# rhasspy/piper

Hardware: AMD Instinct MI355X
Metric: audio samples/sec (higher is better)
Workload: dtype f32

## Files before the change

### piper_amd/csrc/engine.h

```cpp
#pragma once
#include <cstdint>
#include <deque>
#include <list>
#include <map>
#include <string>
#include <unordered_map>
#include <vector>

#include "pe_rt.h"
#include "kernels/params.h"
#include "policy.h"
#include "weights.h"

namespace pe {

struct PackedConv {
  float* wp = nullptr;
  float* wp16 = nullptr;
  float* wpb = nullptr;
  const float* wunscale = nullptr;
  float* wpg4 = nullptr;
  float* bias = nullptr;
  int rows = 0;
  int mtiles = 0;
// ... 178 lines not shown
  int H_, C_, FC_, nh_, dk_, nlayers_, ksz_, window_, hop_, U_;
  std::vector<void*> owned_;
  size_t weight_bytes_ = 0;

  float* emb_ = nullptr;
  float* emb_g_ = nullptr;
  struct EncLayer {
    PackedConv qkv, o, f1, f2;
    float* o16 = nullptr;
    float* qkv16 = nullptr;
    const float *f1p = nullptr, *f2p = nullptr;
    float *relk, *relv, *g1, *b1, *g2, *b2;
  };
  std::vector<EncLayer> enc_;
  PackedConv enc_proj_;
  float* enc_proj16_ = nullptr;
  PackedConv dp_pre_, dp_proj_;
  DdsW dp_dds_;
  struct CFlow {
    float *pre_w, *pre_b;
    DdsW dds;
    PackedConv proj;
    float* proj16 = nullptr;
  };
  std::vector<CFlow> cflows_;
  float ea_m0_ = 0, ea_es0_ = 1;
  float *ea_dev_m_ = nullptr, *ea_dev_logs_ = nullptr;
 public:
  void arena_ready();
 private:
  struct Rcl {
    PackedConv pre, post;
    float *pre16 = nullptr, *post16 = nullptr;
    const float* pre4pad = nullptr;
    std::vector<PackedConv> in, rs;
    std::vector<const float*> rs4;
    int in_off, out_off;
  };
  std::vector<Rcl> rcls_;
  PackedConv dec_pre_;
  struct UpStage {
    PackedConv up;
    int rate, ch;
    std::vector<std::vector<PackedConv>> rb;
    float* last_bias_sum = nullptr;
    struct HostConv { std::vector<float> w; int co = 0, ci = 0, k = 0, dil = 1; const float* bias = nullptr; };
    std::vector<std::vector<HostConv>> rb_host;
    void* mrf_phases = nullptr; float* mrf_w = nullptr;
    float* mrf_wsplit = nullptr; float* mrf_unscale = nullptr; int mrf_wsplit_floats = 0;
    int mrf_wfloats = 0, mrf_cp = 0, mrf_hx = 0;
    std::vector<struct MrfPhase> mrf_ph;
    bool mrf_ok = false, mrf_rb1 = false;
  };
  struct MrfGeo { int ou = 0, N = 0, cu_lo = 0, cu_hi = 0, nleft = 0, nhalo = 0; };
  bool mrf_geo(const UpStage& st, int len_mul, bool tail, MrfGeo& best) const;
  void build_mrf(UpStage& st);
  void mrf(const UpStage& st, View x, View out, const int* lens, int len_mul, int Lmax, bool tail = false);
  bool matrix_bf3_ = false, pack_bf3_now_ = false;
  int matrix_sm_ = 0;
  static bool env_bf3();
 public:
  bool matrix_bf3() const { return matrix_bf3_; }
  int matrix_split_mode() const { return matrix_bf3_ ? matrix_sm_ : -1; }
 private:
  std::vector<UpStage> ups_;
  float* post_w_ = nullptr;
  int post_cin_ = 0;
  struct CondW { float* w; float* b; int rows; };
  CondW cond_dp_{nullptr, nullptr, 0}, cond_dec_{nullptr, nullptr, 0};
  std::vector<CondW> cond_wn_;
  int gin_ = 0, nspk_ = 1;

  int B_ = 0, Tmax_ = 0, Ts_ = 0, Fmax_ = 0, Fs_ = 0, Tg_ = 0, Fg_ = 0;
  bool use_graphs_ = true;
  struct GraphEntry { std::string key; void* exec; long launches; };
  std::list<GraphEntry> graphs_;
  std::unordered_map<std::string, std::list<GraphEntry>::iterator> graph_of_;
  long graph_captures_ = 0;
 public:
  long graph_captures() const { return graph_captures_; }
  size_t graphs_cached() const { return graphs_.size(); }
  static int id_bucket(int T);
  static int frame_bucket(int F);
  void warmup(int max_batch, int max_ids, float frames_per_id, const float* scales, const int64_t* sample, int64_t n_sample);
 private:
  long run_launches_ = 0;
  unsigned long long* d_rng_ = nullptr;
  float scales_[3] = {0.667f, 1.0f, 0.8f};
  std::vector<float> spec_rel_;
  float spec_rel(int b) const { return (size_t)b < spec_rel_.size() ? spec_rel_[b] : 1.f; }
  bool have_noise_w_ = false, have_noise_z_ = false;
  bool drew_w_ = false;
  bool fold_dur_ = false;
  DurP fold_dp_{};
  std::vector<int64_t> id_off_;
  std::vector<int32_t> tlens_h_, frames_h_, dur_h_;
  std::vector<int64_t> sample_off_;
  uint64_t seed_ = 1234, call_ = 0;
  const float* h_noise_z_ = nullptr;
  int64_t h_noise_z_stride_ = 0;

  size_t capA_B_ = 0, capA_T_ = 0, capB_B_ = 0, capB_F_ = 0;
  bool capB_exact_ = false;
  size_t ws_budget_ = 0;
  size_t ws_budget();
  char* wsA_ = nullptr; size_t wsA_bytes_ = 0;
  char* wsB_ = nullptr; size_t wsB_bytes_ = 0;
  int *d_ids_ = nullptr, *d_tlens_ = nullptr, *d_sids_ = nullptr, *d_dur_ = nullptr, *d_cum_ = nullptr,
// ... 56 lines not shown
```

### piper_amd/csrc/engine_launch.cpp

```cpp
#include "engine_internal.h"

namespace pe {


bool Engine::can_group(const PackedConv& pc, int ncols) const {
  if (stage_tiled_) return false;
  const long blocks = (long)((ncols + CFG_BN[pc.cfg] - 1) / CFG_BN[pc.cfg]) * (pc.mtiles * 32 / CFG_BM[pc.cfg]) * B_;
  return pol_.groupable(pc.gate, pc.up != 0, blocks, (pc.ntaps - 1) * pc.dil, pc.Cin);
}
bool Engine::can_group_tiled(const PackedConv& pc, int ncols) const {
  return !pc.gate && pc.up == 0 && route(pc, ncols, EPI_STORE) == ROUTE_TILE && !(matrix_bf3_ && pc.wpb) &&
         !pol_.one_tap_direct(pc.gate, false, pc.ntaps, pc.Cin) && (pc.ntaps - 1) * pc.dil <= 128;
}
static int tile_cfg_of(int cfg) { return cfg == CFG_C ? CFG_C : CFG_S; }
void Engine::group_begin(bool tiled) {
  grouping_ = true;
  group_tiled_ = tiled;
  group_cfg_ = -1;
  group_.clear();
  group_flops_ = group_bytes_ = 0;
}
void Engine::group_end() {
  grouping_ = false;
  if (group_.empty()) return;
// ... 206 lines not shown
    const int BM = BF3_BM[bc], BN = BF3_BN[bc];
    const int HALO = p.xhalo <= 64 ? 64 : 128;
    const int nbuf = pc.nchunks == 1 ? 1 : 2;
    const int nterm = matrix_sm_ == 2 ? 3 : 2;
    const size_t smem = (size_t)nbuf * nterm * 64 * ((BN + HALO + 63) / 64 * 64);
    dim3 grid((ncols + BN - 1) / BN, pc.mtiles * 32 / BM, B_);
    int kh = -1;
    if (prof_level_ >= 2) {
      char nm[96];
      snprintf(nm, sizeof(nm), "conv_split_kernel<%d,%s,%s,%d>", matrix_sm_, (pc.gate && bc == 1) ? "1,4,2,1" : bnames[bc],
               pc.gate ? "true" : "false", HALO);
      kh = kbegin(krow(std::string(nm)), kflops, kbytes);
    }
    launch::conv_bf3(matrix_sm_, bc, pc.gate, HALO, grid, smem, ls_, p);
    kend(kh);
    return;
  }
  if (pol_.one_tap_direct(pc.gate, epi == EPI_CONVT, pc.ntaps, pc.Cin)) {
    const dim3 grid((ncols + 63) / 64, (pc.mtiles + 1) / 2, B_);
    int kh = -1;
    if (prof_level_ >= 2) {
      char nm[96];
      int n = snprintf(nm, sizeof(nm), "conv1x1_kernel<1>");
      if (pol_.prof_sites) snprintf(nm + n, sizeof(nm) - n, "|%dx%dx%d e%d L%d", pc.rows, pc.Cin, pc.ntaps, epi, len_mul);
      kh = kbegin(krow(std::string(nm)), kflops, kbytes);
    }
    launch::conv1x1(grid, ls_, p);
    kend(kh);
    return;
  }
  if (cfg == CFG_A) cfg = pc.gate ? CFG_G : CFG_S;
  else if (cfg == CFG_B && !pc.gate) cfg = CFG_S;
  const int BM = CFG_BM[cfg], BN = CFG_BN[cfg];
  const int ntile = (ncols + BN - 1) / BN, mblocks = pc.mtiles * 32 / BM;
  const int tpb = pol_.tiles_per_workgroup();
  p.tpb = tpb;
  dim3 grid((ntile + tpb - 1) / tpb, mblocks, B_);
  if (p.xhalo > 128) throw std::runtime_error("conv halo (kernel-1)*dilation > 128 is not supported");
  const int nbuf = (tpb == 1 && pc.nchunks == 1) ? 1 : 2;
  const int HALO = p.xhalo <= 64 ? 64 : 128;
  const size_t smem = (size_t)nbuf * KC * ((BN + HALO + 63) / 64 * 64) * sizeof(float);
  static const char* knames[] = {"2,2,2,2,8", "1,4,2,1,16", "1,4,1,1,16", "2,2,1,1,16", "2,2,2,1,16", "1,4,1,2,16", "1,4,2,2,8"};
  int kh = -1;
  if (prof_level_ >= 2) {
    char nm[96];
    int n = snprintf(nm, sizeof(nm), "conv_mfma_kernel<%s,%s,%d>", knames[cfg], pc.gate ? "true" : "false", HALO);
    if (pol_.prof_sites) snprintf(nm + n, sizeof(nm) - n, "|%dx%dx%d d%d e%d L%d", pc.rows, pc.Cin, pc.ntaps, pc.dil, epi, len_mul);
    kh = kbegin(krow(std::string(nm)), kflops, kbytes);
  }
  launch::conv_tile(cfg, pc.gate, HALO, grid, smem, ls_, p);
  kend(kh);
}

bool Engine::mrf_geo(const UpStage& st, int len_mul, bool tail, MrfGeo& best) const {
  const int CP = st.mrf_cp, NCG = CP == 32 ? 8 : 4, HU = CP == 32 ? 1 : 2;
  const int OUMAX = CP == 32 ? 4 : 3;
  const int hx = st.mrf_hx, hxa = rup(hx, 16);
  auto geo = [&](int ou, MrfGeo& g) {
    g.ou = ou; g.N = 16 * NCG * ou;
    if (hxa + g.N + hx > mrf_ws(CP, ou)) return false;
    g.cu_lo = (hxa - hx) / 16; g.cu_hi = (hxa + g.N + hx + 15) / 16;
    g.nleft = hxa / 16 - g.cu_lo; g.nhalo = g.cu_hi - g.cu_lo - g.N / 16;
    return g.nhalo <= NCG * HU;
  };
  best = MrfGeo{};
  double best_cost = 0;
  MrfGeo forced;
  const int force = (pol_.mrf_ou >= 1 && pol_.mrf_ou <= OUMAX && geo((int)pol_.mrf_ou, forced)) ? (int)pol_.mrf_ou : 0;
  for (int ou = 1; ou <= OUMAX; ++ou) {
    MrfGeo g;
    if ((force && ou != force) || !geo(ou, g)) continue;
    double wgs = 0;
    const int stride = tail ? g.N - (POST_K - 1) : g.N;
    for (int b = 0; b < B_; ++b) wgs += (double)(((long)frames_h_[b] * len_mul + stride - 1) / stride);
    double work = 0, taps = 0;
    for (auto& P : st.mrf_ph) {
      const int lo = (hxa - P.e) / 16, hi = (hxa + g.N + P.e + 15) / 16;
      work += (double)(hi - lo) * 16 * P.ntaps;
      taps += P.ntaps;
    }
    double cost = std::ceil(wgs / 256.0) * (work + 16.0 * taps);
    if (ou == 4) cost *= 1.06;
    if (!best.ou || cost < best_cost) { best = g; best_cost = cost; }
  }
  return best.ou != 0;
}

void Engine::mrf(const UpStage& st, View x, View out, const int* lens, int len_mul, int Lmax, bool tail) {
  const int CP = st.mrf_cp, HU = CP == 32 ? 1 : 2;
  const int hx = st.mrf_hx, hxa = rup(hx, 16);
  MrfGeo best;
  if (!mrf_geo(st, len_mul, tail, best)) throw std::runtime_error("internal: no mrf_kernel geometry for this stage");
  MrfP p{};
  p.x = x.p; p.x_bs = x.bs; p.x_cs = x.cs;
  p.out = out.p; p.o_bs = out.bs; p.o_cs = out.cs;
  p.lens = lens; p.len_mul = len_mul;
  p.phases = static_cast<const MrfPhase*>(st.mrf_phases); p.nphases = (int)st.mrf_ph.size();
  p.wstream = st.mrf_w; p.wfloats = st.mrf_wfloats;
  p.C = st.ch; p.N = best.N; p.wcols = hxa + best.N + hx; p.hxa = hxa; p.cu_lo = best.cu_lo; p.cu_hi = best.cu_hi;
  p.nleft = best.nleft; p.nhalo = best.nhalo;
  p.slope = 0.1f;
  p.alpha = 1.0f / (float)st.rb.size();
  p.stride = best.N; p.n0off = 0;
  p.post_w = nullptr; p.audio = nullptr; p.a_bs = 0; p.absmax = nullptr; p.post_slope = 0.01f;
  if (tail) {
    p.stride = best.N - (POST_K - 1); p.n0off = (POST_K - 1) / 2;
    p.post_w = post_w_; p.audio = audio_; p.a_bs = Ss_; p.absmax = absmax_;
  }
  double kflops = 0, kbytes = 0;
  if (prof_level_ >= 2) {
    double cols = 0;
    for (int b = 0; b < B_; ++b) cols += (double)frames_h_[b] * len_mul;
    double macs = 0;
    for (auto& cv : st.rb)
      for (auto& c : cv) macs += c.macs_per_col;
    kflops = 2.0 * macs * cols;
    kbytes = 8.0 * st.ch * cols + 4.0 * st.mrf_wfloats;
    if (tail) {
      kflops += 2.0 * cols * st.ch * POST_K;
      kbytes = 4.0 * (st.ch + 1) * cols + 4.0 * st.mrf_wfloats;
    }
  }
  dim3 grid((Lmax + p.stride - 1) / p.stride, B_);
  char nm[64];
  const bool split = matrix_bf3_ && pol_.mrf_split && st.mrf_wsplit != nullptr && matrix_sm_ < 2;
  if (split) {
    p.wstream = st.mrf_wsplit; p.wfloats = st.mrf_wsplit_floats; p.wunscale = st.mrf_unscale;
    snprintf(nm, sizeof(nm), "mrf_split_kernel<%d,%d,%d,%d>", matrix_sm_, CP, best.ou, HU);
  } else {
    snprintf(nm, sizeof(nm), "mrf_kernel<%d,%d,%d>", CP, best.ou, HU);
  }
  const int kh = prof_level_ >= 2 ? kbegin(krow(std::string(nm)), kflops, kbytes) : -1;
  if (split) launch::mrf_split(matrix_sm_, CP, best.ou, grid, ls_, p);
  else launch::mrf(CP, best.ou, grid, ls_, p);
  kend(kh);
}

size_t Engine::attn_smem(int T, bool global_scores) const {
  const int SP = rup(T, 64) + 1, VS = dk_ + 1 + (dk_ & 1);
  return ((global_scores ? 0 : (size_t)ATT_QB * SP) + (size_t)ATT_KCH * VS + (size_t)dk_ * ATT_QB +
          (size_t)2 * (2 * window_ + 1) * dk_ + 4 * ATT_QB * 16) * sizeof(float);
}
bool Engine::attn_scores_global(int T) const { return pol_.attn_long || attn_smem(T, false) > (size_t)160 * 1024; }

void Engine::layer_norm(View in, View out, const float* g, const float* b, int C, const int* lens, int Lmax) {
  LnP p;
  p.in = in.p; p.i_bs = in.bs; p.i_cs = in.cs;
  p.out = out.p; p.o_bs = out.bs; p.o_cs = out.cs;
  p.gamma = g; p.beta = b;
  p.lens = lens; p.C = C;
  if (C > LN_COLS * 32) throw std::runtime_error("LayerNorm over more than 256 channels is not supported");
  dim3 grid((Lmax + LN_COLS - 1) / LN_COLS, B_);
  const int kh = kbegin(prof_level_ >= 2 ? krow("ln_kernel") : 0, 0.0, 4.0 * 2.0 * C * (lens == d_tlens_ ? cols_ids_ : cols_frames_));
  launch::layer_norm(grid, stream_, p);
  kend(kh);
}

void Engine::dds_params(const DdsW& d, View in, View out, View tmp, const DdsOpt* opt, std::vector<DdsP>& list) {
  int dil = 1;
  const int n = (int)d.c1x1.size();
  View cur = in;
  for (int i = 0; i < n; ++i) {
    const View dst = ((n - 1 - i) & 1) ? tmp : out;
    if (dst.p == cur.p) throw std::runtime_error("internal: DDSConv buffer aliasing");
    DdsP p{};
    if (opt && i == 0 && opt->pre_z) {
      p.pre_z = opt->pre_z; p.pre_z_bs = opt->pre_z_bs; p.pre_w = opt->pre_w; p.pre_b = opt->pre_b;
    }
    p.z_scale = opt ? opt->z_scale : nullptr;
    if (opt && i == n - 1 && opt->post_w16) {
      p.post_w16 = opt->post_w16; p.post_w4 = w4_of(opt->post_w16); p.post_bias = opt->post_bias; p.post_rows = opt->post_rows;
      p.post_out = opt->post_out.p; p.po_bs = opt->post_out.bs; p.po_cs = opt->post_out.cs;
      p.zin = opt->zin; p.zin_bs = opt->zin_bs; p.z_cs = opt->z_cs; p.c0 = opt->c0; p.c1 = opt->c1;
      p.zout = opt->zout; p.zout_bs = opt->zout_bs;
      p.inv_sqrt_h = 1.0f / std::sqrt((float)H_);
    }
    p.x = cur.p; p.x_bs = cur.bs; p.x_cs = cur.cs;
    p.out = dst.p; p.o_bs = dst.bs; p.o_cs = dst.cs;
// ... 193 lines not shown
```

### piper_amd/csrc/kernels/mrf.h

```cpp
#pragma once
#include "../pe_rt.h"
#include "params.h"
#include "conv_common.h"

namespace pe {

template <int V> struct pe_int { static constexpr int value = V; };



template <int NVM, int NDS, int K>
__device__ __forceinline__ void mrf_interleave() {
  if constexpr (NVM + NDS > 0) {
    PE_SCHED_GROUP(0x8, K);
    if constexpr (NVM > 0) {
      PE_SCHED_GROUP(0x20, 1);
      mrf_interleave<NVM - 1, NDS, K>();
    } else {
      PE_SCHED_GROUP(0x100, 1);
      mrf_interleave<0, NDS - 1, K>();
    }
  }
}

// ... 22 lines not shown
  const int l15 = lane & 15, lq = lane >> 4;
  const int ms0 = (wv % NRG) * MSW, cg = wv / NRG;
  const int g0 = n0 - p.hxa;
  const float slope = p.slope;
  const int C = p.C;
  const int wcols = p.wcols;

  const pe_rowsrc wd = pe_make_row(p.wstream, p.wfloats);
  const int wlane = ms0 * 512 + lane * 4;
  const int wlast = PE_UNIFORM(p.wfloats - STEPF);
  auto load_a = [&](int woff, f32x4 (&a)[MSW][2]) {
    woff = woff < wlast ? woff : wlast;
#pragma unroll
    for (int m = 0; m < MSW; ++m)
#pragma unroll
      for (int q = 0; q < 2; ++q) a[m][q] = pe_row_load4_so(wd, wlane + (m * 2 + q) * 256, woff);
  };
  f32x4 aA[MSW][2], aB[MSW][2];
  int wnext = 0;
  load_a(wnext, aA);
  wnext += STEPF;
  {
    const int* gp = reinterpret_cast<const int*>(p.phases);
    for (int i = tid; i < p.nphases * 12; i += NT) tph[i] = gp[i];
    if (tid < MRF_PAD) { sm[tid] = 0.f; bufs[2 * bufsz + tid] = 0.f; }
  }

  const float* xb = p.x + (long)b * p.x_bs;
  auto stage_x = [&]() {
    constexpr int NCC = (WS + 63) / 64, RPW = CP / NW;
    float v[RPW][NCC];
#pragma unroll
    for (int i = 0; i < RPW; ++i) {
      const int row = wv + NW * i;
      const pe_rowsrc rd = pe_make_row(xb + (long)row * p.x_cs, row < C ? L : 0);
#pragma unroll
      for (int j = 0; j < NCC; ++j) v[i][j] = pe_row_load(rd, (lane + 64 * j < wcols) ? g0 + lane + 64 * j : -1);
    }
#pragma unroll
    for (int i = 0; i < RPW; ++i)
#pragma unroll
      for (int j = 0; j < NCC; ++j) {
        const int c = lane + 64 * j;
        if (c < WS) bufs[(wv + NW * i) * WS + c] = pe_lrelu(v[i][j], slope);
      }
  };

  f32x4 acc[MSW][UPW], rawc[MSW][UPW], tot[MSW][OU];
  int cu[UPW];
  {
    const int cuo0 = p.hxa / 16, nout = p.N / 16;
#pragma unroll
    for (int u = 0; u < OU; ++u) cu[u] = cuo0 + cg + NCG * u;
#pragma unroll
    for (int v = 0; v < HU; ++v) {
      const int h = cg + NCG * v;
      cu[OU + v] = h >= p.nhalo ? -1 : (h < p.nleft ? p.cu_lo + h : cuo0 + nout + (h - p.nleft));
    }
#pragma unroll
    for (int m = 0; m < MSW; ++m) {
#pragma unroll
      for (int u = 0; u < UPW; ++u)
#pragma unroll
        for (int r = 0; r < 4; ++r) rawc[m][u][r] = 0.f;
#pragma unroll
      for (int u = 0; u < OU; ++u)
#pragma unroll
        for (int r = 0; r < 4; ++r) tot[m][u][r] = 0.f;
    }
  }
  const pe_rowsrc xd = pe_make_row(xb, C * p.x_cs);
  constexpr int SK = CP == 64 ? 6 : 7;
  PE_STAMP(SK, 0);
  stage_x();
  PE_STAMP(SK, 1);

  for (int ph = 0; ph < p.nphases; ++ph) {
    __syncthreads();
    MrfPhase P;
    {
      const int* t = tph + ph * 12;
      const unsigned lo = PE_UNIFORM((unsigned)t[0]), hi = PE_UNIFORM((unsigned)t[1]);
      P.bias = reinterpret_cast<const float*>(((unsigned long long)hi << 32) | lo);
      P.ntaps = PE_UNIFORM(t[2]); P.dil = PE_UNIFORM(t[3]); P.e = PE_UNIFORM(t[4]);
      P.src = PE_UNIFORM(t[5]); P.dst = PE_UNIFORM(t[6]); P.flags = PE_UNIFORM(t[7]);
    }
    if (P.flags & MRF_RESTAGE) {
      stage_x();
      __syncthreads();
    }
    if (P.flags & MRF_INIT) {
#pragma unroll
      for (int u = 0; u < UPW; ++u) {
        const int g = g0 + 16 * cu[u] + l15;
        int voff = (cu[u] >= 0 && g >= 0 && g < L) ? 4 * lq * p.x_cs + g : 0x3fffffff;
        PE_OPAQUE(voff);
#pragma unroll
        for (int m = 0; m < MSW; ++m) {
          const int vm = (C == CP || (ms0 + m) * 16 + 4 * lq < C) ? voff : 0x3fffffff;
#pragma unroll
          for (int r = 0; r < 4; ++r) rawc[m][u][r] = pe_row_load_so(xd, vm, ((ms0 + m) * 16 + r) * p.x_cs);
        }
      }
    }
    const pe_rowsrc bd = pe_make_row(P.bias, P.bias ? C : 0);
    float bz[MSW][4];
#pragma unroll
    for (int m = 0; m < MSW; ++m)
#pragma unroll
      for (int r = 0; r < 4; ++r) bz[m][r] = pe_row_load(bd, (ms0 + m) * 16 + 4 * lq + r);
    const int hh = P.dil * (P.ntaps - 1) / 2;
    const int wlo = p.hxa - P.e, whi = p.hxa + p.N + P.e;
    bool act[UPW];
#pragma unroll
    for (int u = 0; u < UPW; ++u) {
      act[u] = cu[u] >= 0 && 16 * cu[u] < whi && 16 * cu[u] + 16 > wlo;
#pragma unroll
      for (int m = 0; m < MSW; ++m)
#pragma unroll
        for (int r = 0; r < 4; ++r) acc[m][u][r] = 0.f;
    }
    const float* src = bufs + P.src * bufsz;
    if (ph < 7) PE_STAMP(SK, 2 + 3 * ph);
    auto k_loop = [&](auto maskc) {
      constexpr int MASK = decltype(maskc)::value;
      const int nsteps = NCH * P.ntaps;
      const float* ub[UPW];
#pragma unroll
      for (int u = 0; u < UPW; ++u) ub[u] = src + lq * WS + l15 + 16 * (cu[u] < 0 ? 0 : cu[u]) - hh;
      auto read_b = [&](int soff, float (&bv)[UPW][8]) {
#pragma unroll
        for (int u = 0; u < UPW; ++u)
          if (u < OU || ((MASK >> (u - OU)) & 1)) {
            const float* bp = ub[u] + soff;
#pragma unroll
            for (int s8 = 0; s8 < 8; ++s8) bv[u][s8] = bp[4 * s8 * WS];
          }
      };
      auto mma = [&](const f32x4 (&a)[MSW][2], const float (&bv)[UPW][8]) {
#pragma unroll
        for (int s8 = 0; s8 < 8; ++s8)
#pragma unroll
          for (int u = 0; u < UPW; ++u)
            if (u < OU || ((MASK >> (u - OU)) & 1)) {
#pragma unroll
              for (int m = 0; m < MSW; ++m) acc[m][u] = pe_mfma_16x16x4(a[m][s8 >> 2][s8 & 3], bv[u][s8], acc[m][u]);
            }
      };
      int ntap = 0, nchunk = 0;
      auto advance = [&]() -> int {
        if (++ntap == P.ntaps) { ntap = 0; if (++nchunk == NCH) nchunk = 0; }
        return PE_UNIFORM(nchunk * KC * WS + ntap * P.dil);
      };
      constexpr int NU = OU + ((MASK & 1) ? 1 : 0) + ((MASK & 2) ? 1 : 0);
      constexpr int NMF = 8 * MSW * NU, NVM = 2 * MSW, NDS = 4 * NU;
      if constexpr (MRF_HALF_B<CP, OU, HU>::value) {
        auto read_bh = [&](int soff, int h, float (&bv)[UPW][4]) {
#pragma unroll
          for (int u = 0; u < UPW; ++u)
            if (u < OU || ((MASK >> (u - OU)) & 1)) {
              const float* bp = ub[u] + soff;
#pragma unroll
              for (int s4 = 0; s4 < 4; ++s4) bv[u][s4] = bp[4 * (4 * h + s4) * WS];
            }
        };
        auto mma_h = [&](const f32x4 (&a)[MSW][2], int h, const float (&bv)[UPW][4]) {
#pragma unroll
          for (int s4 = 0; s4 < 4; ++s4)
#pragma unroll
            for (int u = 0; u < UPW; ++u)
              if (u < OU || ((MASK >> (u - OU)) & 1)) {
#pragma unroll
                for (int m = 0; m < MSW; ++m) acc[m][u] = pe_mfma_16x16x4(a[m][h][s4], bv[u][s4], acc[m][u]);
              }
        };
        constexpr int KH0 = (NMF / 2) / (NVM + NDS / 2 + 1), KH1 = (NMF / 2) / (NDS / 2 + 1);
        float b0[UPW][4], b1[UPW][4];
        int cur = 0;
        read_bh(0, 0, b0);
        int st = 0;
        for (; st + 1 < nsteps; st += 2) {
          PE_SCHED_FENCE();
          load_a(wnext, aB);
          read_bh(cur, 1, b1);
          wnext += STEPF;
          mma_h(aA, 0, b0);
          mrf_interleave<NVM, NDS / 2, KH0>();
          PE_SCHED_FENCE();
          cur = advance();
          read_bh(cur, 0, b0);
          mma_h(aA, 1, b1);
          mrf_interleave<0, NDS / 2, KH1>();
          PE_SCHED_FENCE();
          load_a(wnext, aA);
          read_bh(cur, 1, b1);
          wnext += STEPF;
          mma_h(aB, 0, b0);
          mrf_interleave<NVM, NDS / 2, KH0>();
          PE_SCHED_FENCE();
          cur = advance();
          read_bh(cur, 0, b0);
          mma_h(aB, 1, b1);
          mrf_interleave<0, NDS / 2, KH1>();
          PE_SCHED_FENCE();
        }
        if (st < nsteps) {
          load_a(wnext, aB);
          read_bh(cur, 1, b1);
          wnext += STEPF;
          mma_h(aA, 0, b0);
          mrf_interleave<NVM, NDS / 2, KH0>();
          PE_SCHED_FENCE();
          mma_h(aA, 1, b1);
          PE_SCHED_FENCE();
#pragma unroll
          for (int m = 0; m < MSW; ++m)
#pragma unroll
            for (int q = 0; q < 2; ++q) aA[m][q] = aB[m][q];
        }
      } else {
      constexpr int KI = NMF / (NVM + NDS + 1);
      float bA[UPW][8], bB[UPW][8];
      read_b(0, bA);
      int st = 0;
      for (; st + 1 < nsteps; st += 2) {
        PE_SCHED_FENCE();
        load_a(wnext, aB);
        read_b(advance(), bB);
        wnext += STEPF;
        mma(aA, bA);
        mrf_interleave<NVM, NDS, KI>();
        PE_SCHED_FENCE();
        load_a(wnext, aA);
        read_b(advance(), bA);
        wnext += STEPF;
        mma(aB, bB);
        mrf_interleave<NVM, NDS, KI>();
        PE_SCHED_FENCE();
      }
      if (st < nsteps) {
        load_a(wnext, aB);
        wnext += STEPF;
        mma(aA, bA);
        mrf_interleave<NVM, 0, KI>();
        PE_SCHED_FENCE();
#pragma unroll
        for (int m = 0; m < MSW; ++m)
#pragma unroll
          for (int q = 0; q < 2; ++q) aA[m][q] = aB[m][q];
      }
      }
    };
    {
      int mask = 0;
#pragma unroll
      for (int v = 0; v < HU; ++v) mask |= act[OU + v] ? (1 << v) : 0;
      mask = PE_UNIFORM(mask);
      if (HU == 1) {
        if (mask) k_loop(pe_int<1>{}); else k_loop(pe_int<0>{});
      } else {
        switch (mask) {
          case 0: k_loop(pe_int<0>{}); break;
          case 1: k_loop(pe_int<1>{}); break;
          case 2: k_loop(pe_int<2>{}); break;
          default: k_loop(pe_int<3>{}); break;
        }
      }
    }
    if (ph < 7) PE_STAMP(SK, 3 + 3 * ph);
    float* dstb = bufs + (P.dst < 0 ? 0 : P.dst) * bufsz;
#pragma unroll
    for (int u = 0; u < UPW; ++u)
      if (act[u]) {
        const int col = 16 * cu[u] + l15;
        const int g = g0 + col;
        const bool inside = g >= 0 && g < L;
#pragma unroll
        for (int m = 0; m < MSW; ++m) {
          f32x4 v;
#pragma unroll
          for (int r = 0; r < 4; ++r) {
            float t = acc[m][u][r] + bz[m][r];
            if (P.flags & MRF_RES) t += rawc[m][u][r];
            v[r] = inside ? t : 0.f;
          }
          if (P.flags & MRF_KEEP) rawc[m][u] = v;
          if (u < OU && (P.flags & MRF_FINAL)) {
#pragma unroll
            for (int r = 0; r < 4; ++r) tot[m][u < OU ? u : 0][r] += v[r];
          }
          if (P.dst >= 0) {
#pragma unroll
            for (int r = 0; r < 4; ++r) dstb[((ms0 + m) * 16 + 4 * lq + r) * WS + col] = pe_lrelu(v[r], slope);
          }
        }
        if (ph == 4 && u < 4) PE_STAMP(SK, 20 + u);
      }
    if (ph < 7) PE_STAMP(SK, 4 + 3 * ph);
  }
  if (p.post_w == nullptr) {
    float* ob = p.out + (long)b * p.o_bs;
#pragma unroll
    for (int u = 0; u < OU; ++u) {
      const int g = g0 + 16 * cu[u] + l15;
      if (g >= L) continue;
#pragma unroll
      for (int m = 0; m < MSW; ++m)
#pragma unroll
        for (int r = 0; r < 4; ++r) {
          const int row = (ms0 + m) * 16 + 4 * lq + r;
          if (row < C) ob[(long)row * p.o_cs + g] = tot[m][u][r] * p.alpha;
        }
    }
    return;
  }
  __syncthreads();
  float* mb = bufs;
  float* part = bufs + bufsz;
#pragma unroll
  for (int u = 0; u < OU; ++u) {
    const int col = 16 * cu[u] + l15;
#pragma unroll
    for (int m = 0; m < MSW; ++m)
#pragma unroll
      for (int r = 0; r < 4; ++r) mb[((ms0 + m) * 16 + 4 * lq + r) * WS + col] = pe_lrelu(tot[m][u][r] * p.alpha, p.post_slope);
  }
  __syncthreads();
  static_assert(POST_CG * POST_CU == 32 && POST_OPT == 4 && POST_K == 7, "tail mapping: 4 channel groups x 128 threads x 4 samples");
  const int nsamp = p.N - (POST_K - 1);
  {
    const int pg = PE_UNIFORM(tid >> 7), ct = tid & 127;
    if (4 * ct < nsamp) {
      float a4[POST_OPT];
#pragma unroll
      for (int o = 0; o < POST_OPT; ++o) a4[o] = 0.f;
#pragma unroll
      for (int cc = 0; cc < POST_CU; ++cc) {
        const int c = pg * POST_CU + cc;
        if (c < C) {
          const float* rp = mb + c * WS + p.hxa + 4 * ct;
          const f32x4 v0 = *reinterpret_cast<const f32x4*>(rp), v1 = *reinterpret_cast<const f32x4*>(rp + 4);
          const float v[POST_OPT + POST_K - 1] = {v0[0], v0[1], v0[2], v0[3], v1[0], v1[1], v1[2], v1[3], rp[8], rp[9]};
          const float* wc = p.post_w + c * POST_K;
#pragma unroll
          for (int k = 0; k < POST_K; ++k) {
            const float wk = wc[k];
#pragma unroll
            for (int o = 0; o < POST_OPT; ++o) a4[o] = fmaf(wk, v[o + k], a4[o]);
          }
        }
      }
#pragma unroll
      for (int o = 0; o < POST_OPT; ++o) part[pg * p.N + 4 * ct + o] = a4[o];
    }
  }
  __syncthreads();
  float pk = 0.f;
  if (tid < nsamp) {
    float sum = 0.f;
#pragma unroll
    for (int g = 0; g < POST_CG; ++g) sum += part[g * p.N + tid];
    const float y = tanhf(sum);
    const int n = n0 + (POST_K - 1) / 2 + tid;
    if (n < L) {
      p.audio[(long)b * p.a_bs + n] = y;
      pk = fabsf(y);
    }
  }
  for (int o = 32; o >= 1; o >>= 1) pk = fmaxf(pk, __shfl_xor(pk, o));
  float* wmax = part + POST_CG * p.N;
  if (lane == 0) wmax[wv] = pk;
  __syncthreads();
  if (tid == 0) {
    float m = wmax[0];
// ... 8 lines not shown
```

### piper_amd/csrc/kernels/params.h

```cpp
#pragma once
#include <cstddef>

namespace pe {

static constexpr int KC = 32;
enum Epi { EPI_STORE = 0, EPI_RESADD = 1, EPI_GATE = 2, EPI_WNRS = 3, EPI_SUBFROM = 4,
           EPI_ACCUM = 5, EPI_CONVT = 6 };
enum Act { ACT_NONE = 0, ACT_RELU = 1 };
struct ConvP {
  const float* x; long x_bs; int x_cs;
  const float* wp;
  const float* wp16;
  const float* wpb;
  const float* wunscale;
  const float* wpg4;
  const float* bias;
  const float* bias2; int bias2_bs;
  float* out; long o_bs; int o_cs;
  const float* res; long r_bs; int r_cs;
  float* out2; long o2_bs; int o2_cs;
  const int* lens; int len_mul;
  int Cin, rows;
  int nchunks;
  int ntaps, dil, padl;
// ... 131 lines not shown
  const unsigned long long* h_rng; const int* h_lens; const int* h_sids; const float* h_scales; const int* h_ids;
  int* d_lens; int* d_sids; float* d_scales;
  float* draw_out; long draw_stride; int draw_rows, draw_cols;
};

static constexpr int MAX_FRAMES = 60000;
struct DurP {
  const float* z0; long z_bs; float m0, es0;
  const float* scales;
  const int* lens; int* dur; int* cum; int d_bs; int* frames; float* logw_out;
  int* frames_host; int* frames_clamped; int frame_cap;
};
static constexpr int RNG_PITCH = 65536;
static inline unsigned randn_blocks(long rows, int cols) { return (unsigned)(rows * ((cols + 1023) / 1024)); }
struct RegP {
  const float* stats; long s_bs; int s_cs;
  const int* cum; int d_bs;
  const int* tlens; const int* frames;
  float* noise; long n_bs; int n_cs;
  const float* scales;
  float* out; long o_bs; int o_cs;
  int C;
  unsigned* absmax;
  const unsigned long long* rng; int gen;
  DurP dur; int fold;
};
static constexpr int REG_MAXT = 4096;

static constexpr int POST_K = 7, POST_OPT = 4, POST_CU = 8, POST_CG = 4, POST_SPB = 64 * POST_OPT;

enum { MRF_RES = 1, MRF_KEEP = 2, MRF_FINAL = 4, MRF_INIT = 8, MRF_RESTAGE = 16 };
struct MrfPhase {
  const float* bias;
  int ntaps, dil;
  int e;
  int src, dst;
  int flags;
  int pad[4];
};
static_assert(sizeof(MrfPhase) == 48, "MrfPhase is read as 12 ints");
struct MrfP {
  const float* x; long x_bs; int x_cs;
  float* out; long o_bs; int o_cs;
  const int* lens; int len_mul;
  const MrfPhase* phases; int nphases;
  const float* wstream; int wfloats;
  const float* wunscale;
  int C;
  int N;
  int wcols;
  int hxa;
  int cu_lo, cu_hi;
  int nleft, nhalo;
  float slope, alpha;
  int stride, n0off;
  const float* post_w; float* audio; long a_bs; unsigned* absmax; float post_slope;
};
static constexpr int MRF_NW = 8, MRF_PAD = 128, MRF_MAXPH = 24;
static constexpr int mrf_ws(int cp, int ou = 1) { return cp == 32 ? (ou >= 4 ? 624 : 528) : 304; }
static constexpr size_t mrf_smem_bytes(int cp, int ou = 1) {
  return ((size_t)2 * MRF_PAD + (size_t)2 * cp * mrf_ws(cp, ou) + MRF_MAXPH * 12) * sizeof(float);
}

}
```

### piper_amd/csrc/policy.cpp

```cpp
#include "policy.h"

#include <cerrno>
#include <cstdio>
#include <cstdlib>
#include <cstring>
#include <mutex>
#include <stdexcept>
#include <string>

namespace pe {

static const LaunchPolicy::Knob kKnobs[] = {
    {"PIPER_HIP_MRF", &LaunchPolicy::mrf, 0, 2, "fused MRF stage kernel: 0 off (conv by conv), 1 by the measured policy (ResBlock2 stages always; ResBlock1 stages on 32 channels up to PIPER_HIP_MRF_MAXF frames per call), 2 wherever it applies"},
    {"PIPER_HIP_MRF_MAXF", &LaunchPolicy::mrf_maxf, 0, 1L << 40, "batch frames up to which a 32-channel ResBlock1 stage runs in the fused kernel (mode 1)"},
    {"PIPER_HIP_MRF_OU", &LaunchPolicy::mrf_ou, 0, 4, "force the output units per wave of mrf_kernel (1..4) instead of the cost model; ignored when the width does not fit"},
    {"PIPER_HIP_MRF_TAIL", &LaunchPolicy::mrf_tail, 0, 1, "generator tail inside the last stage's mrf_kernel (0: separate conv_post_kernel)"},
    {"PIPER_HIP_MRF_SPLIT", &LaunchPolicy::mrf_split, 0, 1, "matrix modes bf16x3 / f16x3: the fused MRF stage kernel on the 16-bit matrix pipe with split operands (mrf_split_kernel) wherever a fused stage applies; 0 = the f32 fused kernel below PIPER_HIP_BF3_MINF frames, conv by conv on the 16-bit pipe above"},
    {"PIPER_HIP_BF3_MINF", &LaunchPolicy::bf3_minf, 0, 1L << 40, "split matrix modes without a fused 16-bit stage kernel (bf16x6, or PIPER_HIP_MRF_SPLIT=0): batch frames from which the <= 64-channel MRF stages run conv by conv on the 16-bit pipe"},
    {"PIPER_HIP_SPLITK_MAX", &LaunchPolicy::splitk_max, 0, 1L << 40, "tile-workgroup count below which a conv goes to the split-K kernels (0: always the tiled kernel)"},
    {"PIPER_HIP_SPLITK16", &LaunchPolicy::splitk16, 0, 3, "16-column split-K form: 0 off, 1 gate convs, 2 + long-K plain convs, 3 everywhere"},
    {"PIPER_HIP_WIDE_SPLITK", &LaunchPolicy::wide_splitk, 0, 2, "12-wave split-K: 0 off, 1 WN gate conv, 2 always"},
    {"PIPER_HIP_TPB", &LaunchPolicy::tpb, 0, 64, "tiled kernel: column tiles walked by one workgroup (0 = 1)"},
    {"PIPER_HIP_GROUP_MRF", &LaunchPolicy::group_mrf, 0, 2, "sibling resblock convs of a wider small stage as grouped launches (one-utterance calls): 0 off, 2 without the K-concatenated last step"},
    {"PIPER_HIP_GROUP_MAXB", &LaunchPolicy::group_maxb, 0, 1L << 40, "64 x 64 tiles of one conv of a stage below which the grouped sibling launches of a single utterance take the split-K kernels (the tiled grouped launches from there on)"},
    {"PIPER_HIP_GROUP_TILED", &LaunchPolicy::group_tiled, 0, 1, "sibling resblock convs of a stage that runs the tiled kernel as grouped launches (conv_mfma_group_kernel) while one conv is at most 2048 tile workgroups (8 per CU): 0 = one launch per conv"},
    {"PIPER_HIP_COLCHAIN", &LaunchPolicy::colchain, 0, 2, "colchain_kernel / lngemm_kernel: 0 off, 1 up to 4096 ids / 8192 frames per call, 2 always"},
    {"PIPER_HIP_COL4", &LaunchPolicy::col4, 0, 2, "4-column forms of the 192-channel chains: 0 off, 1 up to PIPER_HIP_COL4_MAXC ids (2048 frames for the flow's launches) per call, 2 always"},
    {"PIPER_HIP_COL4_MAXC", &LaunchPolicy::col4_maxc, 0, 1L << 40, "ids per call up to which the 4-column chains are used"},
    {"PIPER_HIP_FFN", &LaunchPolicy::ffn, 0, 1, "the encoder FFN as one launch (ffn_kernel) wherever the 4-column chains run: 0 = conv by conv"},
    {"PIPER_HIP_ATTNO", &LaunchPolicy::attno, 0, 1, "attention + conv_o + norm_layers_1 as one launch (attno_kernel) wherever the 4-column chains run: 0 = attn_kernel + colchain4_kernel"},
    {"PIPER_HIP_ATTN4", &LaunchPolicy::attn4, 0, 2, "attention + conv_o + norm_layers_1 on 4-query workgroups (attn4_kernel) in place of attno_kernel: 0 off, 1 for calls whose longest utterance has up to PIPER_HIP_ATTN4_MAXC ids, 2 wherever attno_kernel applies"},
    {"PIPER_HIP_ATTN4_MAXC", &LaunchPolicy::attn4_maxc, 0, 1L << 40, "ids of the longest utterance of a call up to which attention runs on 4-query workgroups"},
    {"PIPER_HIP_FUSE_DP", &LaunchPolicy::fuse_dp, 0, 1, "ConvFlow.pre / proj / spline fused into the DDSConv layer launches"},
    {"PIPER_HIP_SPEC", &LaunchPolicy::spec, 0, 1, "speculative stage-B sizing / whole utterance as one graph for <= 4 utterances per call"},
    {"PIPER_HIP_SPEC_EXPECT", &LaunchPolicy::spec_expect, 0, 1, "speculative graphs planned for the expected frame counts (0: for the bucket capacity)"},
    {"PIPER_HIP_PCM_ZC", &LaunchPolicy::pcm_zc, 0, 1, "PCM written straight into pinned host memory by pcm16_kernel (0: one copy per utterance behind the graph)"},
    {"PIPER_HIP_IDS_ZC", &LaunchPolicy::ids_zc, 0, 1, "phoneme ids, lengths and speaker ids read straight from the pinned host block by embed_kernel, up to 65536 padded ids per call (0: one host-to-device copy in front of the graph)"},
    {"PIPER_HIP_NO_GRAPH", &LaunchPolicy::no_graph, 0, 1, "launch kernels directly instead of replaying hipGraphs"},
    {"PIPER_HIP_GRAPHS", &LaunchPolicy::graphs, 1, 4096, "hipGraphs kept per engine (least recently used evicted one at a time)"},
    {"PIPER_HIP_CONVT_VEC", &LaunchPolicy::convt_vec, 0, 1, "polyphase up-conv: a lane's four accumulator rows leave as one 16-byte store (stride a multiple of 4) or two 8-byte stores (stride 2) of consecutive output samples; 0: one 4-byte store per phase"},
    {"PIPER_HIP_XCD", &LaunchPolicy::xcd, -1, 32, "XCDs the dispatch round-robins over, for the XCD-aware tile orders (-1 = probed at engine creation, 0 = tiles in workgroup order)"},
    {"PIPER_HIP_XCD_FFN", &LaunchPolicy::xcd_ffn, 0, 1, "ffn_kernel deals (column tile, slice) to the XCDs slice-major, so an XCD's L2 holds two slices' weights instead of all sixteen (0: blockIdx order)"},
    {"PIPER_HIP_STACK_PRE", &LaunchPolicy::stack_pre, 0, 1, "small calls of the 192-channel voices: enc_p.proj and dp.pre (both read the last LayerNorm's output) as one lngemm4_kernel launch over the stacked matrix (0: two launches)"},
    {"PIPER_HIP_CHAIN_RS", &LaunchPolicy::chain_rs, 0, 1, "small calls of the 192-channel voices: the last WN layer's res/skip conv (skip rows only) in front of the coupling layer's post + pre chain launch, colchain4_kernel<true> (0: a launch of its own)"},
    {"PIPER_HIP_GATE4", &LaunchPolicy::gate4, 0, 2, "short calls: the WN gate conv over 192 channels on 64-row x 12-column workgroups with the 4x4x1 MFMA (gate4_kernel) up to 640 workgroups: 0 off (16-column split-K form), 2 wherever the split-K route applies"},
    {"PIPER_HIP_GATE_HALF", &LaunchPolicy::gate_half, 0, 1, "short one-utterance calls (up to 128 whole-group workgroups): the WN gate conv on half a 32-channel group per workgroup, six waves with the whole K range in flight, twice the workgroups (0: whole groups on twelve waves)"},
    {"PIPER_HIP_CONV1X1", &LaunchPolicy::conv1x1, 0, 1, "batched one-tap convs (q/k/v, WN res/skip, coupling pre/post, proj) through conv1x1_kernel, B operand straight from global memory (0: the tiled kernel)"},
    {"PIPER_HIP_WS_BUDGET_MB", &LaunchPolicy::ws_budget_mb, 0, 1048576, "MiB of device memory the workspace of one pipeline half may take (0: a third of the device's memory): capacities grow only inside it, a call that does not fit by itself is an error"},
    {"PIPER_HIP_ATTN_LONG", &LaunchPolicy::attn_long, 0, 1, "attention score slabs in global memory (attn_long_kernel) at every length, also in place of attno_kernel (tests): by default only utterances whose 32 x T slab does not fit LDS (more than ~830 ids) take that form"},
    {"PIPER_HIP_PROF_SITES", &LaunchPolicy::prof_sites, 0, 1, "level-2 profile rows of the tiled conv kernel per conv shape (tuning aid)"},
    {"PIPER_HIP_DEBUG_KEEP", &LaunchPolicy::debug_keep, 0, 1, "test hook: keep z_p for pe_debug_tensor"},
    {"PIPER_HIP_DEBUG_POISON", &LaunchPolicy::debug_poison, 0, 1, "test hook: activation workspaces are filled with NaN bit patterns when allocated (no kernel may read what the call did not write)"},
};

const LaunchPolicy::Knob* LaunchPolicy::knobs(int* n) {
  if (n) *n = (int)(sizeof(kKnobs) / sizeof(kKnobs[0]));
  return kKnobs;
}

void LaunchPolicy::read_env() {
  for (const Knob& k : kKnobs) {
    const char* t = getenv(k.env);
    if (!t || !*t) continue;
    errno = 0;
    char* end = nullptr;
    const long v = strtol(t, &end, 10);
    if (errno || end == t || *end)
      throw std::runtime_error(std::string(k.env) + "=" + t + ": not an integer (" + k.doc + ")");
// ... 37 lines not shown
```

### piper_amd/csrc/policy.h

```cpp
#pragma once
#include <cstddef>

namespace pe {

struct LaunchPolicy {
  long mrf = 1;
  long mrf_maxf = 1100;
  long mrf_ou = 0;
  long mrf_tail = 1;
  long mrf_split = 1;
  long bf3_minf = 1100;
  long splitk_max = 96;
  long splitk16 = 2;
  long wide_splitk = 1;
  long tpb = 0;
  long group_mrf = 1;
  long group_maxb = 160;
  long group_tiled = 1;
  long colchain = 1;
  long col4 = 1;
  long col4_maxc = 1024;
  long ffn = 1;
  long attno = 1;
  long attn4 = 1;
  long attn4_maxc = 512;
  long fuse_dp = 1;
  long spec = 1;
  long spec_expect = 1;
  long pcm_zc = 1;
  long ids_zc = 1;
  long no_graph = 0;
  long graphs = 256;
  long convt_vec = 1;
  long xcd = -1;
  long xcd_ffn = 1;
  long stack_pre = 1;
  long chain_rs = 1;
  long gate4 = 1;
  long gate_half = 1;
  long conv1x1 = 1;
  long ws_budget_mb = 0;
  long attn_long = 0;
  long prof_sites = 0;
  long debug_keep = 0;
  long debug_poison = 0;

  static constexpr long colchain_max_ids = 4096, colchain_max_frames = 8192;
  static constexpr long col4_max_frames = 2048;
  static constexpr long ffn_max_cols = 2048;
  static constexpr int spec_max_batch = 4;
  static constexpr long ids_zc_max = 65536;
  static constexpr long group_max_blocks64 = 700;
  static constexpr long group_tiled_max_blocks = 2048;

  struct Knob { const char* env; long LaunchPolicy::*field; long lo, hi; const char* doc; };
  static const Knob* knobs(int* n);
  void read_env();
  static const char* describe();
  static int matrix_mode_env();
  static bool matrix_bf3_env() { return matrix_mode_env() >= 0; }

// ... 50 lines not shown
```

Measured before the change: 119.7 million.

## Allow half-width MRF windows where half the column groups own one fewer unit

Adds intermediate tile widths N = 16*(NCG*OU - NCG/2) to the fused MRF kernel's cost model. In these windows half the waves skip their last output unit via masked k_loop variants. The aim is to better fit the workgroup count to the GPU when the launch is small (at most 256 workgroups in default mode 1) and reduce wasted padded columns. The cost is more kernel instantiations and some load imbalance between waves.

```diff
diff --git a/piper_amd/csrc/engine.h b/piper_amd/csrc/engine.h
--- a/piper_amd/csrc/engine.h
+++ b/piper_amd/csrc/engine.h
@@ -254,8 +254,8 @@
     std::vector<struct MrfPhase> mrf_ph;
     bool mrf_ok = false, mrf_rb1 = false;
   };
-  struct MrfGeo { int ou = 0, N = 0, cu_lo = 0, cu_hi = 0, nleft = 0, nhalo = 0; };
-  bool mrf_geo(const UpStage& st, int len_mul, bool tail, MrfGeo& best) const;
+  struct MrfGeo { int ou = 0, N = 0, cu_lo = 0, cu_hi = 0, nleft = 0, nhalo = 0, nlive = 0; };
+  bool mrf_geo(const UpStage& st, int len_mul, bool tail, bool partial, MrfGeo& best) const;
   void build_mrf(UpStage& st);
   void mrf(const UpStage& st, View x, View out, const int* lens, int len_mul, int Lmax, bool tail = false);
   bool matrix_bf3_ = false, pack_bf3_now_ = false;
diff --git a/piper_amd/csrc/engine_launch.cpp b/piper_amd/csrc/engine_launch.cpp
--- a/piper_amd/csrc/engine_launch.cpp
+++ b/piper_amd/csrc/engine_launch.cpp
@@ -282,12 +282,12 @@
   kend(kh);
 }
 
-bool Engine::mrf_geo(const UpStage& st, int len_mul, bool tail, MrfGeo& best) const {
+bool Engine::mrf_geo(const UpStage& st, int len_mul, bool tail, bool partial, MrfGeo& best) const {
   const int CP = st.mrf_cp, NCG = CP == 32 ? 8 : 4, HU = CP == 32 ? 1 : 2;
   const int OUMAX = CP == 32 ? 4 : 3;
   const int hx = st.mrf_hx, hxa = rup(hx, 16);
-  auto geo = [&](int ou, MrfGeo& g) {
-    g.ou = ou; g.N = 16 * NCG * ou;
+  auto geo = [&](int ou, MrfGeo& g, bool half = false) {
+    g.ou = ou; g.N = 16 * (NCG * ou - (half ? NCG / 2 : 0)); g.nlive = half ? NCG / 2 : NCG;
     if (hxa + g.N + hx > mrf_ws(CP, ou)) return false;
     g.cu_lo = (hxa - hx) / 16; g.cu_hi = (hxa + g.N + hx + 15) / 16;
     g.nleft = hxa / 16 - g.cu_lo; g.nhalo = g.cu_hi - g.cu_lo - g.N / 16;
@@ -297,12 +297,16 @@
   double best_cost = 0;
   MrfGeo forced;
   const int force = (pol_.mrf_ou >= 1 && pol_.mrf_ou <= OUMAX && geo((int)pol_.mrf_ou, forced)) ? (int)pol_.mrf_ou : 0;
-  for (int ou = 1; ou <= OUMAX; ++ou) {
+  for (int cand = 2; cand <= 2 * OUMAX + 1; ++cand) {
+    const int ou = cand / 2;
+    const bool half = !(cand & 1);
     MrfGeo g;
-    if ((force && ou != force) || !geo(ou, g)) continue;
+    if ((half && (!partial || ou < 2)) || (force && ou != force) || !geo(ou, g, half)) continue;
+    if (partial && pol_.mrf_half == 2 && !half && ou >= 2) continue;
     double wgs = 0;
     const int stride = tail ? g.N - (POST_K - 1) : g.N;
     for (int b = 0; b < B_; ++b) wgs += (double)(((long)frames_h_[b] * len_mul + stride - 1) / stride);
+    if (half && pol_.mrf_half == 1 && wgs > 256) continue;
     double work = 0, taps = 0;
     for (auto& P : st.mrf_ph) {
       const int lo = (hxa - P.e) / 16, hi = (hxa + g.N + P.e + 15) / 16;
@@ -320,7 +324,8 @@
   const int CP = st.mrf_cp, HU = CP == 32 ? 1 : 2;
   const int hx = st.mrf_hx, hxa = rup(hx, 16);
   MrfGeo best;
-  if (!mrf_geo(st, len_mul, tail, best)) throw std::runtime_error("internal: no mrf_kernel geometry for this stage");
+  const bool split = matrix_bf3_ && pol_.mrf_split && st.mrf_wsplit != nullptr && matrix_sm_ < 2;
+  if (!mrf_geo(st, len_mul, tail, !split && pol_.mrf_half != 0, best)) throw std::runtime_error("internal: no mrf_kernel geometry for this stage");
   MrfP p{};
   p.x = x.p; p.x_bs = x.bs; p.x_cs = x.cs;
   p.out = out.p; p.o_bs = out.bs; p.o_cs = out.cs;
@@ -328,7 +333,7 @@
   p.phases = static_cast<const MrfPhase*>(st.mrf_phases); p.nphases = (int)st.mrf_ph.size();
   p.wstream = st.mrf_w; p.wfloats = st.mrf_wfloats;
   p.C = st.ch; p.N = best.N; p.wcols = hxa + best.N + hx; p.hxa = hxa; p.cu_lo = best.cu_lo; p.cu_hi = best.cu_hi;
-  p.nleft = best.nleft; p.nhalo = best.nhalo;
+  p.nleft = best.nleft; p.nhalo = best.nhalo; p.nlive = best.nlive;
   p.slope = 0.1f;
   p.alpha = 1.0f / (float)st.rb.size();
   p.stride = best.N; p.n0off = 0;
@@ -353,7 +358,6 @@
   }
   dim3 grid((Lmax + p.stride - 1) / p.stride, B_);
   char nm[64];
-  const bool split = matrix_bf3_ && pol_.mrf_split && st.mrf_wsplit != nullptr && matrix_sm_ < 2;
   if (split) {
     p.wstream = st.mrf_wsplit; p.wfloats = st.mrf_wsplit_floats; p.wunscale = st.mrf_unscale;
     snprintf(nm, sizeof(nm), "mrf_split_kernel<%d,%d,%d,%d>", matrix_sm_, CP, best.ou, HU);
diff --git a/piper_amd/csrc/kernels/mrf.h b/piper_amd/csrc/kernels/mrf.h
--- a/piper_amd/csrc/kernels/mrf.h
+++ b/piper_amd/csrc/kernels/mrf.h
@@ -98,6 +98,7 @@
     const int cuo0 = p.hxa / 16, nout = p.N / 16;
 #pragma unroll
     for (int u = 0; u < OU; ++u) cu[u] = cuo0 + cg + NCG * u;
+    if (cg >= p.nlive) cu[OU - 1] = -1;
 #pragma unroll
     for (int v = 0; v < HU; ++v) {
       const int h = cg + NCG * v;
@@ -169,7 +170,8 @@
     const float* src = bufs + P.src * bufsz;
     if (ph < 7) PE_STAMP(SK, 2 + 3 * ph);
     auto k_loop = [&](auto maskc) {
-      constexpr int MASK = decltype(maskc)::value;
+      constexpr int MASK = decltype(maskc)::value & 3;
+      constexpr int NO = (decltype(maskc)::value & 4) ? OU - 1 : OU;
       const int nsteps = NCH * P.ntaps;
       const float* ub[UPW];
 #pragma unroll
@@ -177,7 +179,7 @@
       auto read_b = [&](int soff, float (&bv)[UPW][8]) {
 #pragma unroll
         for (int u = 0; u < UPW; ++u)
-          if (u < OU || ((MASK >> (u - OU)) & 1)) {
+          if (u < NO || (u >= OU && ((MASK >> (u - OU)) & 1))) {
             const float* bp = ub[u] + soff;
 #pragma unroll
             for (int s8 = 0; s8 < 8; ++s8) bv[u][s8] = bp[4 * s8 * WS];
@@ -188,7 +190,7 @@
         for (int s8 = 0; s8 < 8; ++s8)
 #pragma unroll
           for (int u = 0; u < UPW; ++u)
-            if (u < OU || ((MASK >> (u - OU)) & 1)) {
+            if (u < NO || (u >= OU && ((MASK >> (u - OU)) & 1))) {
 #pragma unroll
               for (int m = 0; m < MSW; ++m) acc[m][u] = pe_mfma_16x16x4(a[m][s8 >> 2][s8 & 3], bv[u][s8], acc[m][u]);
             }
@@ -198,13 +200,13 @@
         if (++ntap == P.ntaps) { ntap = 0; if (++nchunk == NCH) nchunk = 0; }
         return PE_UNIFORM(nchunk * KC * WS + ntap * P.dil);
       };
-      constexpr int NU = OU + ((MASK & 1) ? 1 : 0) + ((MASK & 2) ? 1 : 0);
+      constexpr int NU = NO + ((MASK & 1) ? 1 : 0) + ((MASK & 2) ? 1 : 0);
       constexpr int NMF = 8 * MSW * NU, NVM = 2 * MSW, NDS = 4 * NU;
       if constexpr (MRF_HALF_B<CP, OU, HU>::value) {
         auto read_bh = [&](int soff, int h, float (&bv)[UPW][4]) {
 #pragma unroll
           for (int u = 0; u < UPW; ++u)
-            if (u < OU || ((MASK >> (u - OU)) & 1)) {
+            if (u < NO || (u >= OU && ((MASK >> (u - OU)) & 1))) {
               const float* bp = ub[u] + soff;
 #pragma unroll
               for (int s4 = 0; s4 < 4; ++s4) bv[u][s4] = bp[4 * (4 * h + s4) * WS];
@@ -215,7 +217,7 @@
           for (int s4 = 0; s4 < 4; ++s4)
 #pragma unroll
             for (int u = 0; u < UPW; ++u)
-              if (u < OU || ((MASK >> (u - OU)) & 1)) {
+              if (u < NO || (u >= OU && ((MASK >> (u - OU)) & 1))) {
 #pragma unroll
                 for (int m = 0; m < MSW; ++m) acc[m][u] = pe_mfma_16x16x4(a[m][h][s4], bv[u][s4], acc[m][u]);
               }
@@ -302,7 +304,18 @@
 #pragma unroll
       for (int v = 0; v < HU; ++v) mask |= act[OU + v] ? (1 << v) : 0;
       mask = PE_UNIFORM(mask);
-      if (HU == 1) {
+      if (cu[OU - 1] < 0) {
+        if (HU == 1) {
+          if (mask) k_loop(pe_int<5>{}); else k_loop(pe_int<4>{});
+        } else {
+          switch (mask) {
+            case 0: k_loop(pe_int<4>{}); break;
+            case 1: k_loop(pe_int<5>{}); break;
+            case 2: k_loop(pe_int<6>{}); break;
+            default: k_loop(pe_int<7>{}); break;
+          }
+        }
+      } else if (HU == 1) {
         if (mask) k_loop(pe_int<1>{}); else k_loop(pe_int<0>{});
       } else {
         switch (mask) {
@@ -349,7 +362,7 @@
 #pragma unroll
     for (int u = 0; u < OU; ++u) {
       const int g = g0 + 16 * cu[u] + l15;
-      if (g >= L) continue;
+      if (cu[u] < 0 || g >= L) continue;
 #pragma unroll
       for (int m = 0; m < MSW; ++m)
 #pragma unroll
@@ -366,6 +379,7 @@
 #pragma unroll
   for (int u = 0; u < OU; ++u) {
     const int col = 16 * cu[u] + l15;
+    if (cu[u] < 0) continue;
 #pragma unroll
     for (int m = 0; m < MSW; ++m)
 #pragma unroll
diff --git a/piper_amd/csrc/kernels/params.h b/piper_amd/csrc/kernels/params.h
--- a/piper_amd/csrc/kernels/params.h
+++ b/piper_amd/csrc/kernels/params.h
@@ -207,6 +207,7 @@
   int hxa;
   int cu_lo, cu_hi;
   int nleft, nhalo;
+  int nlive;
   float slope, alpha;
   int stride, n0off;
   const float* post_w; float* audio; long a_bs; unsigned* absmax; float post_slope;
diff --git a/piper_amd/csrc/policy.cpp b/piper_amd/csrc/policy.cpp
--- a/piper_amd/csrc/policy.cpp
+++ b/piper_amd/csrc/policy.cpp
@@ -14,6 +14,7 @@
     {"PIPER_HIP_MRF", &LaunchPolicy::mrf, 0, 2, "fused MRF stage kernel: 0 off (conv by conv), 1 by the measured policy (ResBlock2 stages always; ResBlock1 stages on 32 channels up to PIPER_HIP_MRF_MAXF frames per call), 2 wherever it applies"},
     {"PIPER_HIP_MRF_MAXF", &LaunchPolicy::mrf_maxf, 0, 1L << 40, "batch frames up to which a 32-channel ResBlock1 stage runs in the fused kernel (mode 1)"},
     {"PIPER_HIP_MRF_OU", &LaunchPolicy::mrf_ou, 0, 4, "force the output units per wave of mrf_kernel (1..4) instead of the cost model; ignored when the width does not fit"},
+    {"PIPER_HIP_MRF_HALF", &LaunchPolicy::mrf_half, 0, 2, "mrf_kernel (f32): the cost model may also pick windows of N = 16 * (NCG * OU - NCG / 2) columns, half the column groups of waves owning one output unit fewer (0: only N = 16 * NCG * OU; 2: the narrower width wherever OU >= 2, tests)"},
     {"PIPER_HIP_MRF_TAIL", &LaunchPolicy::mrf_tail, 0, 1, "generator tail inside the last stage's mrf_kernel (0: separate conv_post_kernel)"},
     {"PIPER_HIP_MRF_SPLIT", &LaunchPolicy::mrf_split, 0, 1, "matrix modes bf16x3 / f16x3: the fused MRF stage kernel on the 16-bit matrix pipe with split operands (mrf_split_kernel) wherever a fused stage applies; 0 = the f32 fused kernel below PIPER_HIP_BF3_MINF frames, conv by conv on the 16-bit pipe above"},
     {"PIPER_HIP_BF3_MINF", &LaunchPolicy::bf3_minf, 0, 1L << 40, "split matrix modes without a fused 16-bit stage kernel (bf16x6, or PIPER_HIP_MRF_SPLIT=0): batch frames from which the <= 64-channel MRF stages run conv by conv on the 16-bit pipe"},
diff --git a/piper_amd/csrc/policy.h b/piper_amd/csrc/policy.h
--- a/piper_amd/csrc/policy.h
+++ b/piper_amd/csrc/policy.h
@@ -7,6 +7,7 @@
   long mrf = 1;
   long mrf_maxf = 1100;
   long mrf_ou = 0;
+  long mrf_half = 1;
   long mrf_tail = 1;
   long mrf_split = 1;
   long bf3_minf = 1100;
```

After: 121.7 million (median of 6 runs). No clear change (+1.7%).
